# acoustic-warfare/zybo-rt-sampler-image-detection

Measured on AMD Instinct MI355X. Metric: beam-steered frames/sec (64 mics x 256 samples x 101x101 angles), higher is better.
Workload: dtype f32

## Files before the change

include/beamformer_hip.h:

```cpp
#ifndef BEAMFORMER_HIP_H
#define BEAMFORMER_HIP_H

#include <stdbool.h>

#ifdef __cplusplus
extern "C" {
#endif


void pad_delay(float *signal, float *out, int pos_pad);
void miso_pad(float *signals, float *out, int *adaptive_array, int n, int offset);
void miso_pad2(float *signals, float *out, int *adaptive_array, int n, int offset);
void mimo_pad(float *signals, float *image, int *adaptive_array, int n);
void load_coefficients_pad(int *whole_samples, int n);
void load_coefficients_pad2(int *whole_miso, int n);
void unload_coefficients_pad(void);
void unload_coefficients_pad2(void);

void lerp_delay(float *signal, float *out, float h, int pad);
void miso_lerp(float *signals, float *out, int *adaptive_array, int n, int offset);
void mimo_lerp(float *signals, float *image, int *adaptive_array, int n);
void load_coefficients_lerp(float *delays, int n);
void unload_coefficients_lerp(void);

// ... 32 lines not shown


enum bf_algo {
    BF_PAD = 0,
    BF_LERP = 1,
    BF_HYBRID = 2,
    BF_FIR_NAIVE = 3,
    BF_FIR_VEC = 4
};

int bf_configure(int n_microphones, int n_samples, int max_res_x, int max_res_y, int n_taps);
int bf_configure_from_json(const char *path);
void bf_get_config(int out[5]);

const char *bf_last_error(void);
void bf_clear_error(void);

int bf_gpu_available(void);
int bf_last_das_variant(void);
int bf_last_das_reloads(long long *changes, long long *steps);
int bf_sweep_order(const int *whole, int n_dirs, int n_mics, int dir_begin, int dir_end, int dpw, int *order_out);
int bf_read_phase_stamps(unsigned long long *out16, int clear);
int bf_read_wave_stamps(unsigned long long *out128, int clear);
int bf_set_device(int device);

void bf_publish_frame(const float *signals);
int bf_miso_listen_block(float *out, float mic_gain);
int bf_get_steer(int *n_out);

int bf_das_device(int algo, const float *d_signals, int m_total, float *d_images, int image_stride, int frames,
                  const int *adaptive_array, int n, int dir_begin, int dir_end, void *stream);

int bf_miso_device(int algo, const float *d_signals, int m_total, int frames, const int *adaptive_array, int n,
                   const int *d_offsets, int beams, float mic_gain, float *d_out, int out_stride, int *d_status, void *stream);
int bf_peak_offsets_device(const float *d_power, int frames, int image_stride, int n_dirs, int offset_per_dir,
                           int *d_offsets, void *stream);

#define BF_PEAKS_MAX_K 64
int bf_peaks_device(const float *d_power, int frames, int image_stride, int rows, int cols, int radius, int k,
                    float floor_rel, float floor_abs, int offset_per_dir,
                    int *d_offsets, float *d_values, int *d_counts, void *stream);

#define BF_REMOVE_MAX_BEAMS 64
int bf_remove_sources_device(int algo, const float *d_signals, int m_total, int frames, const int *adaptive_array, int n,
                             const int *d_offsets, int beams, const float *d_beams, int beam_stride, float gain,
                             float *d_residual, int *d_status, void *stream);
// ... 153 lines not shown
```

zybo-rt-sampler-image-detection_amd/csrc/beamformer_api.cpp:

```cpp
#include <hip/hip_runtime.h>

#include <algorithm>
#include <chrono>
#include <cmath>
#include <cstdarg>
#include <cstdio>
#include <cstdlib>
#include <cstring>
#include <initializer_list>
#include <limits>
#include <mutex>
#include <string>
#include <thread>
#include <vector>

#include "../../include/beamformer_hip.h"
#include "das_kernels.h"
#include "sweep_order.h"

namespace {

using bf::Algo;

struct Sizes {
// ... 748 lines not shown
{
    if (!need_ptrs("bf_sweep_order", {{whole, "whole"}, {order_out, "order_out"}})) return -1;
    if (n_dirs < 1 || n_mics < 1 || dpw < 1 || dir_begin < 0 || dir_end > n_dirs || dir_begin >= dir_end) {
        set_error("bf_sweep_order: want n_dirs, n_mics, dpw >= 1 and 0 <= dir_begin < dir_end <= n_dirs (got %d, %d, %d, [%d, %d))", n_dirs, n_mics, dpw,
                  dir_begin, dir_end);
        return -1;
    }
    static_assert(sizeof(int) == sizeof(int32_t), "the C-ABI's int tables are int32");
    return bf::sweep_order(reinterpret_cast<const int32_t*>(whole) + (size_t)dir_begin * n_mics, n_mics, dir_end - dir_begin, n_mics, dir_begin, dpw,
                           reinterpret_cast<int32_t*>(order_out), nullptr);
}
int bf_read_phase_stamps(unsigned long long* out16, int clear)
{
    std::lock_guard<std::mutex> lock(S().mu);
    if (!out16 || !ensure_device()) return -1;
    return HIP_OK(hipDeviceSynchronize()) && HIP_OK(bf::read_phase_stamps(out16, clear != 0)) ? 0 : -1;
}
int bf_read_wave_stamps(unsigned long long* out128, int clear)
{
    std::lock_guard<std::mutex> lock(S().mu);
    if (!out128 || !ensure_device()) return -1;
    return HIP_OK(hipDeviceSynchronize()) && HIP_OK(bf::read_wave_stamps(out128, clear != 0)) ? 0 : -1;
}

int bf_gpu_available(void)
{
    int count = 0;
    return (hipGetDeviceCount(&count) == hipSuccess && count > 0) ? 1 : 0;
}

int bf_set_device(int device)
{
    std::lock_guard<std::mutex> lock(S().mu);
    if (S().device_ready && device != S().device) { set_error("bf_set_device: device %d already in use", S().device); return -1; }
    S().device = device;
    return 0;
}


void load_coefficients_pad(int* whole_samples, int n) { (void)load_whole_only(SLOT_PAD, whole_samples, n, "load_coefficients_pad"); }
void unload_coefficients_pad(void) { std::lock_guard<std::mutex> lock(S().mu); S().tab[SLOT_PAD].drop(); }

void load_coefficients_pad2(int* whole_miso, int n)
{
    std::lock_guard<std::mutex> lock(S().mu);
    if (!whole_miso || n < 1) { set_error("load_coefficients_pad2: null or empty table"); return; }
// ... 1134 lines not shown
```

zybo-rt-sampler-image-detection_amd/csrc/das_device.h:

```cpp
#pragma once
#include "das_geometry.h"

namespace bf {

namespace {

struct KArgs {
    long long miso_row;
    int n_mics, m_total, n_samples, n_taps;
    int dir_begin, dir_end, image_stride, image_origin;
    int lead, row_stride, mic_chunk, n_chunks, tile_dirs, n_tiles;
    int scratch_off, srow, pbw;
    int n_is_pow2;
    float inv_n;
    int n_frames;
    int wg_frames, frame_inner;
    long long digest_h_off;
    long long digest_t_off;
    long long digest_o_off;
};

__device__ __forceinline__ void tile_and_frame(const KArgs& a, int* tile, int* frame)
{
    const unsigned id = blockIdx.x;
    if (a.frame_inner) {
        const unsigned x = id & 7u, j = id >> 3;
        *tile = (int)(x + 8u * (j / (unsigned)a.wg_frames));
        *frame = (int)(j % (unsigned)a.wg_frames);
    } else {
        *tile = (int)(id % (unsigned)a.n_tiles);
        *frame = (int)(id / (unsigned)a.n_tiles);
    }
}

#define BF_TABLE_PARAMS                                                                                   \
    const float* __restrict__ signals, float* __restrict__ images, const int32_t* __restrict__ mics,     \
        const int32_t* __restrict__ whole, const float* __restrict__ frac, const float* __restrict__ taps
#define BF_TABLE_ARGS signals, images, mics, whole, frac, taps

__device__ __forceinline__ float wave_sum(float v)
{
#pragma unroll
    for (int off = 32; off > 0; off >>= 1) v += __shfl_xor(v, off, kWave);
    return v;
}

__device__ __forceinline__ void stage_chunk(float* lds, const KArgs& a, const int32_t* __restrict__ mics,
                                            const float* __restrict__ frame, int m0, int mc, int wave, int nwaves, int lane)
{
    const int n = a.n_samples;
    for (int r = wave; r < mc; r += nwaves) {
        const int mic = mics[m0 + r];
        const float* src = frame + (size_t)mic * n;
        float* dst = lds + r * a.row_stride + a.lead;
        if ((n & 3) == 0) {
            const float4* s4 = reinterpret_cast<const float4*>(src);
// ... 193 lines not shown
```

zybo-rt-sampler-image-detection_amd/csrc/das_kernels.h:

```cpp
#pragma once
#include <hip/hip_runtime.h>
#include <stdint.h>

namespace bf {

enum Algo : int {
    ALGO_PAD = 0,
    ALGO_LERP = 1,
    ALGO_HYBRID = 2,
    ALGO_FIR_NAIVE = 3,
    ALGO_FIR_VEC = 4,
    ALGO_COUNT = 5
};

struct DeviceTables {
    const int32_t* whole = nullptr;
    const float* frac = nullptr;
    const float* taps = nullptr;
    int max_whole = 0;
    bool digest_direct = false;
    const int32_t* digest = nullptr;
    long long digest_order_off = 0;
};

// ... 120 lines not shown
hipError_t launch_mvdr_learn(const float* d_signals, int m_total, int frames, int n_samples, const int32_t* d_mics, int n, int seg_first, int seg_hop, int segs,
                             const double* d_window, const double* d_weights, double forget, const double* d_tau, int dirs, const int32_t* d_offsets, int sources,
                             int offset_per_dir, int n_taps, int bin_lo, int bin_hi, double loading, double* d_acc, double* d_mass, int32_t* d_used,
                             double* d_snap, double* d_cov, double* d_chol, double* d_gains, float* d_taps, int32_t* d_status, int32_t* d_fallback,
                             hipStream_t stream);

hipError_t launch_fd_steering(const double* d_tau, const double* d_freq, int n_dirs, int n_mics, int n_bins, float* d_are, float* d_aim, hipStream_t stream);
size_t fd_twiddle_floats(int n_samples, int n_bins);
hipError_t launch_fd_twiddles(int n_samples, int bin_lo, int n_bins, float* d_tw, hipStream_t stream);
hipError_t launch_fd_dft(const float* d_frames, const int32_t* d_mics, int m_total, int n_samples, int n_frames, int n_mics, int bin_lo, int n_bins,
                         const float* d_tw, float* xre_mf, float* xim_mf, float* xre_fm, float* xim_fm, hipStream_t stream);
size_t fd_workspace_floats(int n_rows, int n_dirs, int n_bins);
hipError_t launch_fd_das_power(const float* xre_mf, const float* xim_mf, const float* are, const float* aim, int n_frames, int n_mics, int n_dirs,
                               int n_bins, float* d_power, float* d_work, size_t work_floats, hipStream_t stream);
hipError_t launch_fd_covariance(const float* xre_fm, const float* xim_fm, int n_frames, int n_mics, int n_bins, float* rre, float* rim, hipStream_t stream);
size_t fd_cholesky_workspace_floats(int n_mics, int n_bins);
hipError_t launch_fd_cholesky_inverse(const float* rre, const float* rim, int n_mics, int n_bins, float loading, float* lire_t, float* liim_t,
                                      int* d_status, float* d_work, size_t work_floats, hipStream_t stream);
hipError_t launch_fd_mvdr_power(const float* lire_t, const float* liim_t, const float* are, const float* aim, int n_mics, int n_dirs, int n_bins,
                                float* d_power, float* d_work, size_t work_floats, hipStream_t stream);

hipError_t read_phase_stamps(unsigned long long* out16, bool clear);
hipError_t read_wave_stamps(unsigned long long* out128, bool clear);

hipError_t launch_yolo_decode(const void* const raw[3], const int hs[3], const int ws[3], const int strides[3], const float* anchors,
                              int batch, int nc, int format, float conf_thres, float* d_boxes, float* d_scores, int* d_cls, hipStream_t stream);
hipError_t launch_upsample_concat(const void* a, const void* b, void* out, int B, int H, int W, int ca, int cb, int elem_bytes, hipStream_t stream);
hipError_t launch_sppf_pool(void* buf, int B, int H, int W, int c, int elem_bytes, hipStream_t stream);
hipError_t launch_preprocess_bgr8(const void* frames, void* out, long long pixels, int cpad, int elem_bytes, hipStream_t stream);
int conv_dma_switch(int value);
int conv_f32_mode(int value);
int gemm_f32_mode(int value);
int conv_weight_row(int elem_bytes, int kh, int kw, int c);
hipError_t launch_conv2d_nhwc(int elem_bytes, const void* x, const void* w, const float* bias, void* y, int B, int H, int W, int C, int N, int KH, int KW,
                              int stride, int pad, int act, int ldy, const void* res, int ldr, const void* x2, int c1, int ld1, int ld2, int up1,
                              hipStream_t stream);
hipError_t launch_topk_candidates(const float* d_scores, const float* d_boxes, const int* d_cls, int batch, int total, int K, float* d_top_scores,
                                  float* d_top_boxes, int* d_top_cls, int* d_counts, hipStream_t stream);
hipError_t launch_nms(const float* d_boxes, const float* d_scores, const int* d_cls, const int* d_counts, int batch, int K, float iou_thres,
                      int max_det, unsigned long long* d_mask, float* d_out, int* d_out_count, hipStream_t stream);

}
```

zybo-rt-sampler-image-detection_amd/csrc/das_pair.hip:

```cpp
#include "das_device.h"

namespace bf {

namespace {

namespace copies {


#define BF_P_ACC(n, j, f) [a##n##0] "+v"(acc[j][f][0]), [a##n##1] "+v"(acc[j][f][1])
#define BF_P_PAD_STEP(n0, n1)                                                                             \
    "v_pk_add_f32 %[a" #n0 "0], %[a" #n0 "0], %[s0l]\n\tv_pk_add_f32 %[a" #n0 "1], %[a" #n0 "1], %[s0h]\n\t" \
    "v_pk_add_f32 %[a" #n1 "0], %[a" #n1 "0], %[s1l]\n\tv_pk_add_f32 %[a" #n1 "1], %[a" #n1 "1], %[s1h]\n\t"
#define BF_P_PAD_READ                                                                                     \
    "ds_read_b64 %[s0l], %[ad] offset:0\n\tds_read_b64 %[s0h], %[ad] offset:8\n\t"                         \
    "ds_read_b64 %[s1l], %[ad] offset:%[f0]\n\tds_read_b64 %[s1h], %[ad] offset:%[f8]\n\t"                 \
    "s_waitcnt lgkmcnt(0)\n\t"
#define BF_P_ADDR(e) "v_add_u32 %[ad], %[" #e "], %[lb]\n\t"
#define BF_P_CHECK(n, ep, ec) "s_cmp_lg_u32 %[" #ec "], %[" #ep "]\n\ts_cbranch_scc1 .Lr" #n "_%=\n.Lb" #n "_%=:\n\t"
#define BF_P_STUB(n, ec, READ) ".Lr" #n "_%=:\n\t" BF_P_ADDR(ec) READ "s_branch .Lb" #n "_%=\n"

__device__ __forceinline__ void pair_pad_first(f32x2 (&acc)[8][2][2], Quad& S0, Quad& S1, int eb, int ec, int lbase)
{
    using G = PairGeo;
    int ad;
// ... 11 lines not shown

__device__ __forceinline__ void pair_pad_rest(f32x2 (&acc)[8][2][2], Quad& S0, Quad& S1, const int (&e)[8], int lbase)
{
    using G = PairGeo;
    int ad;
#define BF_P_ACC2(n, j) [a##n##0] "+v"(acc[j][0][0]), [a##n##1] "+v"(acc[j][0][1]), [b##n##0] "+v"(acc[j][1][0]), [b##n##1] "+v"(acc[j][1][1])
#define BF_P_PAD1(n) "v_pk_add_f32 %[a" #n "0], %[a" #n "0], %[s0l]\n\tv_pk_add_f32 %[a" #n "1], %[a" #n "1], %[s0h]\n\t" \
                     "v_pk_add_f32 %[b" #n "0], %[b" #n "0], %[s1l]\n\tv_pk_add_f32 %[b" #n "1], %[b" #n "1], %[s1h]\n\t"
    asm volatile(BF_P_CHECK(2, e1, e2) BF_P_PAD1(2) BF_P_CHECK(3, e2, e3) BF_P_PAD1(3) BF_P_CHECK(4, e3, e4) BF_P_PAD1(4)
                 BF_P_CHECK(5, e4, e5) BF_P_PAD1(5) BF_P_CHECK(6, e5, e6) BF_P_PAD1(6) BF_P_CHECK(7, e6, e7) BF_P_PAD1(7)
                 ".subsection 1\n" BF_P_STUB(2, e2, BF_P_PAD_READ) BF_P_STUB(3, e3, BF_P_PAD_READ) BF_P_STUB(4, e4, BF_P_PAD_READ)
                 BF_P_STUB(5, e5, BF_P_PAD_READ) BF_P_STUB(6, e6, BF_P_PAD_READ) BF_P_STUB(7, e7, BF_P_PAD_READ) "\t.subsection 0"
                 : BF_P_ACC2(2, 2), BF_P_ACC2(3, 3), BF_P_ACC2(4, 4), BF_P_ACC2(5, 5), BF_P_ACC2(6, 6), BF_P_ACC2(7, 7),
                   [s0l] "+v"(S0.lo), [s0h] "+v"(S0.hi), [s1l] "+v"(S1.lo), [s1h] "+v"(S1.hi), [ad] "=&v"(ad)
                 : [e1] "s"(e[1]), [e2] "s"(e[2]), [e3] "s"(e[3]), [e4] "s"(e[4]), [e5] "s"(e[5]), [e6] "s"(e[6]), [e7] "s"(e[7]), [lb] "v"(lbase),
                   [f0] "n"(G::kFoff), [f8] "n"(G::kFoff + 8)
                 : "scc");
#undef BF_P_ACC2
#undef BF_P_PAD1
}

#ifdef BF_STAMPS
__device__ unsigned long long g_stamps[64 * 16];
#define BF_STAMP_DECL unsigned long long st_acc[8] = {0, 0, 0, 0, 0, 0, 0, 0}; unsigned long long st_prev = __builtin_amdgcn_s_memtime();
#define BF_STAMP(k) do { const unsigned long long st_now = __builtin_amdgcn_s_memtime(); st_acc[k] += st_now - st_prev; st_prev = st_now; } while (0)
__device__ unsigned long long g_wave_stamps[64 * 16 * 8];
__device__ unsigned char g_wave_simd[4096 * 16];
#define BF_STAMP_FLUSH do { if (lane == 0) { unsigned long long* gs = g_stamps + 16 * (blockIdx.x & 63); for (int i = 0; i < 8; ++i) atomicAdd(&gs[i], st_acc[i]); atomicAdd(&gs[8], 1ull); \
                            unsigned simd; asm volatile("s_getreg_b32 %0, hwreg(HW_REG_HW_ID, 4, 2)" : "=s"(simd)); \
                            unsigned long long* gw = g_wave_stamps + 128 * (blockIdx.x & 63) + 8 * (wave & 15); \
                            atomicAdd(&gw[0], st_acc[0]); atomicAdd(&gw[1], st_acc[3]); atomicAdd(&gw[2 + (simd & 3)], 1ull); \
                            g_wave_simd[16 * (blockIdx.x & 4095) + (wave & 15)] = (unsigned char)(0x80 | (simd & 3)); } } while (0)
#else
#define BF_STAMP_DECL
#define BF_STAMP(k)
#define BF_STAMP_FLUSH
#endif

template <int ALGO>
__global__ void __launch_bounds__(1024, 4) das_pair_kernel(BF_TABLE_PARAMS, KArgs a)
{
    static_assert(ALGO == ALGO_PAD, "das_pair_kernel: pad (lerp runs das_pair2_kernel)");
    using G = PairGeo;
    constexpr int C = G::kC, RS = G::kRs, LEAD = G::kLead, HC = G::kHalf, W = 16, DW = 8, kGroup = DW * W, kPark = Geo<1>::kPark;
    extern __shared__ __attribute__((aligned(16))) float lds[];
    const int lane = threadIdx.x & (kWave - 1);
    const int wave = __builtin_amdgcn_readfirstlane((int)(threadIdx.x >> 6));
    int tile, fpair;
    tile_and_frame(a, &tile, &fpair);
    const int f0 = 2 * fpair;
    const bool two = f0 + 1 < a.n_frames;
    const int f1 = two ? f0 + 1 : f0;
    const int tile_begin = a.dir_begin + tile * a.tile_dirs;
    if (tile_begin >= a.dir_end) return;
    const int tile_end = min(tile_begin + a.tile_dirs, a.dir_end);
    const int M = a.n_mics, N = a.n_samples;
    const int n_half = M / HC;
    const float* __restrict__ sig0 = signals + (size_t)f0 * a.m_total * N;
    const float* __restrict__ sig1 = signals + (size_t)f1 * a.m_total * N;
    float* __restrict__ img0 = images + (size_t)f0 * a.image_stride;
    float* __restrict__ img1 = images + (size_t)f1 * a.image_stride;
    const int32_t* __restrict__ dig = reinterpret_cast<const int32_t*>(taps);

    const int vmic = (lane < n_half) ? mics[lane * HC + (wave >> 1)] : 0;
    auto fetch = [&](int h) -> float4 {
        const int mic = (h < kWave) ? __builtin_amdgcn_readlane(vmic, h) : mics[h * HC + (wave >> 1)];
        const float* src = ((wave & 1) ? sig1 : sig0) + (size_t)mic * N;
        float4 v = make_float4(0.f, 0.f, 0.f, 0.f);
        if (4 * lane < N) v = *reinterpret_cast<const float4*>(src + 4 * lane);
        return v;
    };
    auto stage = [&](int h, const float4 v, bool wipe) {
        float* row0 = lds + (((h & 1) * W) + wave) * G::kSlot;
        const float py = dpp_prev(v.y), pz = dpp_prev(v.z), pw = dpp_prev(v.w);
        write_copies<C>(row0, RS, LEAD, lane, v, py, pz, pw);
        if (wipe) {
            static_assert((LEAD >> 2) * C <= kWave, "one lane per prefix quad");
            constexpr int PQ = LEAD >> 2;
            if (lane < PQ * C) reinterpret_cast<float4*>(row0 + (lane / PQ) * RS)[lane % PQ] = make_float4(0.f, 0.f, 0.f, 0.f);
        }
    };

    float4 st = fetch(0);
    const int lb = 16 * lane + (int)(unsigned)(size_t)((__attribute__((address_space(3))) char*)lds);
    BF_STAMP_DECL

    for (int g0 = tile_begin; g0 < tile_end; g0 += kGroup) {
        f32x2 acc[DW][2][2];
#pragma unroll
        for (int j = 0; j < DW; ++j)
#pragma unroll
            for (int f = 0; f < 2; ++f) { acc[j][f][0] = f32x2{0.0f, 0.0f}; acc[j][f][1] = f32x2{0.0f, 0.0f}; }

        BF_STAMP(7);
        __syncthreads();
        BF_STAMP(1);
        stage(0, st, true);
        st = fetch(1);
        BF_STAMP(2);
        __syncthreads();
        BF_STAMP(3);

        for (int h = 0; h < n_half; ++h) {
            asm volatile("s_setprio 3");
            if (h + 1 < n_half) {
                stage(h + 1, st, h == 0);
                if (h + 2 < n_half) st = fetch(h + 2);
                else if (g0 + kGroup < tile_end) st = fetch(0);
                BF_STAMP(2);
            }
            const int dw0 = g0 + wave * DW;
            if (dw0 < tile_end) {
                const size_t grp = (size_t)(dw0 - a.dir_begin) / DW;
                const int32_t* __restrict__ et = dig + (grp * M + (size_t)h * HC) * DW;
                struct Entries { int e[DW]; };
                auto request = [&](Entries& t, int m) {
#pragma unroll
                    for (int j = 0; j < DW; ++j) t.e[j] = et[m * DW + j];
                };
// ... 36 lines not shown
            auto park = [&](auto mul_c) {
#pragma unroll
                for (int j = 0; j < DW; ++j) {
                    float* row = lds + (wave * DW + j) * kPark;
                    const f32x2 a0 = acc[j][f][0], a1 = acc[j][f][1];
                    float o0, o1, o2, o3;
                    mic_mean<decltype(mul_c)::value>(a0.x, a0.y, a1.x, a1.y, M, a.inv_n, o0, o1, o2, o3);
                    reinterpret_cast<float4*>(row)[lane] = make_float4(o0 * o0, o1 * o1, o2 * o2, o3 * o3);
                }
            };
            if (__builtin_expect(a.n_is_pow2, 1)) park(std::true_type{}); else park(std::false_type{});
            BF_STAMP(5);
            __syncthreads();
            BF_STAMP(6);
            const int g = wave * kWave + lane;
            const int d = g0 + g;
            if (g < kGroup && d < tile_end && (f == 0 || two)) {
                const int dd = a.digest_o_off != 0 ? dig[a.digest_o_off + (d - a.dir_begin)] : d;
                (f == 0 ? img0 : img1)[dd - a.image_origin] = row_mean_power<false>(lds + g * kPark, N);
            }
        }
    }
    BF_STAMP(7);
    BF_STAMP_FLUSH;
}
#undef BF_P_ACC
#undef BF_P_PAD_STEP
#undef BF_P_PAD_READ
#undef BF_P_ADDR
#undef BF_P_CHECK
#undef BF_P_STUB


#define BF_I_ACC(n, j) [a##n##0] "+v"(acc[j][0]), [a##n##1] "+v"(acc[j][1]), [a##n##2] "+v"(acc[j][2]), [a##n##3] "+v"(acc[j][3])
#define BF_I_READ                                                                                   \
    "ds_read_b128 v[96:99], v120\n\tds_read_b128 v[100:103], v120 offset:1024\n\t"                   \
    "ds_read_b128 v[104:107], v120 offset:%[g0]\n\tds_read_b128 v[108:111], v120 offset:%[g1]\n\ts_waitcnt lgkmcnt(0)\n\t"
#define BF_I_STEP(n, h, mods)                                                                       \
    "v_pk_fma_f32 v[112:113], %[" #h "], v[104:105], v[96:97] " mods "\n\tv_pk_fma_f32 v[114:115], %[" #h "], v[106:107], v[98:99] " mods "\n\t" \
    "v_pk_fma_f32 v[116:117], %[" #h "], v[108:109], v[100:101] " mods "\n\tv_pk_fma_f32 v[118:119], %[" #h "], v[110:111], v[102:103] " mods "\n\t" \
    "v_pk_add_f32 %[a" #n "0], %[a" #n "0], v[112:113]\n\tv_pk_add_f32 %[a" #n "1], %[a" #n "1], v[114:115]\n\t" \
    "v_pk_add_f32 %[a" #n "2], %[a" #n "2], v[116:117]\n\tv_pk_add_f32 %[a" #n "3], %[a" #n "3], v[118:119]\n\t"
#define BF_I_FIRST(h, mods)                                                                         \
    "ds_read_b128 v[96:99], v120\n\tds_read_b128 v[104:107], v120 offset:%[g0]\n\t"                \
    "ds_read_b128 v[100:103], v120 offset:1024\n\tds_read_b128 v[108:111], v120 offset:%[g1]\n\ts_waitcnt lgkmcnt(2)\n\t" \
    "v_pk_fma_f32 v[112:113], %[" #h "], v[104:105], v[96:97] " mods "\n\tv_pk_fma_f32 v[114:115], %[" #h "], v[106:107], v[98:99] " mods "\n\t" \
    "v_pk_add_f32 %[a00], %[a00], v[112:113]\n\tv_pk_add_f32 %[a01], %[a01], v[114:115]\n\ts_waitcnt lgkmcnt(0)\n\t" \
// ... 25 lines not shown
                 : BF_I_ACC(1, 1), BF_I_ACC(2, 2), BF_I_ACC(3, 3), BF_I_ACC(4, 4), BF_I_ACC(5, 5), BF_I_ACC(6, 6), BF_I_ACC(7, 7)
                 : [e0] "s"(e[0]), [e1] "s"(e[1]), [e2] "s"(e[2]), [e3] "s"(e[3]), [e4] "s"(e[4]), [e5] "s"(e[5]), [e6] "s"(e[6]), [e7] "s"(e[7]), [lb] "v"(lbase),
                   [h01] "s"(hp[0]), [h23] "s"(hp[1]), [h45] "s"(hp[2]), [h67] "s"(hp[3]), [g0] "n"(G::kDoff), [g1] "n"(G::kDoff + 1024)
                 : "scc", BF_I_CLOB);
}
#undef BF_I_ACC
#undef BF_I_READ
#undef BF_I_FIRST
#undef BF_I_STEP
#undef BF_I_EVEN
#undef BF_I_ODD
#undef BF_I_CHECK
#undef BF_I_STUB
#undef BF_I_CLOB

template <int ALGO>
__global__ void __launch_bounds__(1024, 4) das_pair2_kernel(BF_TABLE_PARAMS, KArgs a)
{
    static_assert(ALGO == ALGO_LERP, "das_pair2_kernel: lerp (pad runs das_pair_kernel)");
    using G = Pair2Geo;
    constexpr int C = G::kC, RS = G::kRs, LEAD = G::kLead, HC = G::kHalf, W = 16, DW = 8, kGroup = DW * W, kParkHalf = Geo<1>::kParkHalf;
    static_assert(2 * kGroup * kParkHalf <= G::kMc * G::kSlot, "both frames' parked half rows fit the LDS image they alias");
    extern __shared__ __attribute__((aligned(16))) float lds[];
    const int lane = threadIdx.x & (kWave - 1);
    auto lane_id = []() -> int {
        int l;
        asm volatile("v_mbcnt_lo_u32_b32 %0, -1, 0\n\tv_mbcnt_hi_u32_b32 %0, -1, %0" : "=v"(l));
        return l;
    };
    const int wave = __builtin_amdgcn_readfirstlane((int)(threadIdx.x >> 6));
    int tile, fpair;
    tile_and_frame(a, &tile, &fpair);
    const int f0 = 2 * fpair;
    const bool two = f0 + 1 < a.n_frames;
    const int f1 = two ? f0 + 1 : f0;
    const int tile_begin = a.dir_begin + tile * a.tile_dirs;
    if (tile_begin >= a.dir_end) return;
    const int tile_end = min(tile_begin + a.tile_dirs, a.dir_end);
    const int M = a.n_mics, N = a.n_samples;
    const int n_half = M / HC;
    const float* __restrict__ sig0 = signals + (size_t)f0 * a.m_total * N;
    const float* __restrict__ sig1 = signals + (size_t)f1 * a.m_total * N;
    float* __restrict__ img0 = images + (size_t)f0 * a.image_stride;
    float* __restrict__ img1 = images + (size_t)f1 * a.image_stride;
    const int32_t* __restrict__ dig = reinterpret_cast<const int32_t*>(taps);

    const int my_mic = wave & 7, part = wave >> 3;
    constexpr unsigned kHalfBytes = HC * G::kSlot * 4;
    const bool full = N == 256;
    const unsigned row_bytes = 4u * (unsigned)N, hoff_end = (unsigned)n_half * (HC * 4u);
    unsigned voff = min(16u * (unsigned)lane, row_bytes - 16u);
    const bool in_row = 16u * (unsigned)lane < row_bytes;
    const char* mic_ids = reinterpret_cast<const char*>(mics + my_mic);
    unsigned hoff = 0;
    int mic_a = *reinterpret_cast<const int32_t*>(mic_ids);
    struct Staged2 { float4 v0, v1; };
    auto fetch_next = [&]() -> Staged2 {
        const size_t row = (size_t)(unsigned)mic_a * row_bytes;
        const char* r0 = reinterpret_cast<const char*>(sig0) + row;
        const char* r1 = reinterpret_cast<const char*>(sig1) + row;
        asm volatile("" : "+v"(voff));
        Staged2 st;
        st.v0 = *reinterpret_cast<const float4*>(r0 + voff);
        st.v1 = *reinterpret_cast<const float4*>(r1 + voff);
        hoff = hoff + HC * 4u < hoff_end ? hoff + HC * 4u : 0u;
        mic_a = *reinterpret_cast<const int32_t*>(mic_ids + hoff);
        return st;
    };
#define BF_I_DPP " row_mask:0xf bank_mask:0xf bound_ctrl:1\n\t"
    const int lb = 16 * lane + (int)(unsigned)(size_t)((__attribute__((address_space(3))) char*)lds);
    const int row0 = (my_mic * G::kSlot + part * C * RS) * 4 - (int)(unsigned)(size_t)((__attribute__((address_space(3))) char*)lds), row1 = row0 + (int)kHalfBytes;
    auto stage = [&](int row, const Staged2& st) {
        const int ad = 2 * lb + row;
        float4 x = st.v0, y = st.v1;
        if (!full) {
            asm volatile(";BF_STAGE_MASKED");
            x = make_float4(in_row ? x.x : 0.f, in_row ? x.y : 0.f, in_row ? x.z : 0.f, in_row ? x.w : 0.f);
            y = make_float4(in_row ? y.x : 0.f, in_row ? y.y : 0.f, in_row ? y.z : 0.f, in_row ? y.w : 0.f);
        }
        asm volatile("s_cmp_eq_u32 %[part], 0\n\ts_cbranch_scc1 .Lp0_%=\n\t"
                     "v_sub_f32 v98, %[xy], %[xx]\n\tv_sub_f32 v99, %[yy], %[yx]\n\t"
                     "v_sub_f32_dpp v104, %[xx], %[xw] wave_shl:1" BF_I_DPP "v_sub_f32_dpp v105, %[yx], %[yw] wave_shl:1" BF_I_DPP
                     "v_sub_f32 v100, %[xz], %[xy]\n\tv_sub_f32 v101, %[yz], %[yy]\n\t"
                     "v_sub_f32 v102, %[xw], %[xz]\n\tv_sub_f32 v103, %[yw], %[yz]\n"
                     ".Lst_%=:\n\t"
                     "v_mov_b32_dpp v96, v104 wave_shr:1" BF_I_DPP "v_mov_b32_dpp v97, v105 wave_shr:1" BF_I_DPP
                     "ds_write_b128 %[ad], v[98:101] offset:%[c0]\n\tds_write_b128 %[ad], v[102:105] offset:%[c0] + 16\n\t"
                     "ds_write_b128 %[ad], v[96:99] offset:%[c1]\n\tds_write_b128 %[ad], v[100:103] offset:%[c1] + 16\n\t"
                     ".subsection 1\n"
                     ".Lp0_%=:\n\t;BF_STAGE_PART0\n\t"
                     "v_mov_b32 v104, %[xw]\n\tv_mov_b32 v105, %[yw]\n\tv_mov_b32 v98, %[xx]\n\tv_mov_b32 v99, %[yx]\n\t"
                     "v_mov_b32 v100, %[xy]\n\tv_mov_b32 v101, %[yy]\n\tv_mov_b32 v102, %[xz]\n\tv_mov_b32 v103, %[yz]\n\t"
                     "s_branch .Lst_%=\n\t.subsection 0"
                     : : [xx] "v"(x.x), [xy] "v"(x.y), [xz] "v"(x.z), [xw] "v"(x.w), [yx] "v"(y.x), [yy] "v"(y.y), [yz] "v"(y.z), [yw] "v"(y.w),
                         [ad] "v"(ad), [part] "s"(part), [c0] "n"(2 * LEAD * 4), [c1] "n"((RS + 2 * LEAD) * 4)
                     : "memory", "scc", "v96", "v97", "v98", "v99", "v100", "v101", "v102", "v103", "v104", "v105");
    };
#undef BF_I_DPP
    auto wipe_prefix = [&]() {
        constexpr int PQ = LEAD >> 1;
        static_assert(2 * PQ <= kWave, "one lane per prefix quad of two rows");
        const int l = lane_id();
        if (l < 2 * PQ) {
            float* rows = lds + my_mic * G::kSlot + part * C * RS;
            float4* q = reinterpret_cast<float4*>(rows + (l < PQ ? 0 : RS)) + (l < PQ ? l : l - PQ);
            q[0] = make_float4(0.f, 0.f, 0.f, 0.f);
            *reinterpret_cast<float4*>(reinterpret_cast<char*>(q) + kHalfBytes) = make_float4(0.f, 0.f, 0.f, 0.f);
        }
    };

    BF_STAMP_DECL
    Staged2 st = fetch_next();

    for (int g0 = tile_begin; g0 < tile_end; g0 += kGroup) {
        f32x2 acc[DW][4];
#pragma unroll
        for (int j = 0; j < DW; ++j)
#pragma unroll
            for (int q = 0; q < 4; ++q) acc[j][q] = f32x2{0.0f, 0.0f};

        BF_STAMP(7);
        __syncthreads();
        BF_STAMP(1);
        wipe_prefix();
        stage(row0, st);
        st = fetch_next();
        BF_STAMP(2);
        __syncthreads();
        BF_STAMP(3);

        const int dw0 = g0 + wave * DW;
        const bool busy = dw0 < tile_end;
        const size_t grp = busy ? (size_t)(dw0 - a.dir_begin) / DW : 0;
        const int32_t* __restrict__ etg = dig + grp * M * DW;
        const float* __restrict__ htg = reinterpret_cast<const float*>(dig) + a.digest_h_off + grp * M * DW;
        int row_next = row1;
        for (int h = 0; h < n_half; ++h) {
            asm volatile("s_setprio 3");
            asm volatile(";BF_STAGE_BEGIN");
            if (h + 1 < n_half) {
                stage(row_next, st);
                row_next = row0 + row1 - row_next;
                st = fetch_next();
                BF_STAMP(2);
            }
            asm volatile(";BF_STAGE_END");
// ... 14 lines not shown
                    constexpr int K = decltype(kc)::value, K2 = (K + 2) % 3;
                    const Entries& cur = E[K];
                    pair2_first(acc, cur.e[0], cur.hp[0], lb);
                    request(E[K2], m + 2);
                    pair2_rest(acc, cur.e, cur.hp, lb);
                };
                using I0 = std::integral_constant<int, 0>; using I1 = std::integral_constant<int, 1>; using I2 = std::integral_constant<int, 2>;
                static_assert(HC == 8, "eight mics, the three entry sets in rotation");
                mic(0, I0{}); mic(1, I1{});
                asm volatile("s_setprio 2");
                mic(2, I2{}); mic(3, I0{});
                asm volatile("s_setprio 1");
                mic(4, I1{}); mic(5, I2{});
                asm volatile("s_setprio 0");
                mic(6, I0{}); mic(7, I1{});
                __builtin_amdgcn_s_waitcnt(0xC07F);
            }
            BF_STAMP(0);
            __syncthreads();
            BF_STAMP(h + 1 < n_half ? 3 : 4);
        }
        asm volatile("s_setprio 0");

        auto power_pass = [&](auto mul_c) __attribute__((always_inline)) {
        constexpr bool MUL = decltype(mul_c)::value;
        if constexpr (MUL) asm volatile(";BF_POWER_POW2"); else asm volatile(";BF_POWER_DIV");
        int wv = wave;
        asm volatile("" : "+s"(wv));
        float sum = 0.0f;
#pragma unroll
        for (int r = 0; r < 2; ++r) {
            if (r == 1) {
                __syncthreads();
                BF_STAMP(4);
            }
            {
                auto squares = [&](int j, f32x2& s0, f32x2& s1) __attribute__((always_inline)) {
                    if constexpr (MUL) {
                        const f32x2 inv2 = {a.inv_n, a.inv_n};
                        s0 = acc[j][2 * r] * inv2; s1 = acc[j][2 * r + 1] * inv2;
                    } else {
                        float o0, o1, o2, o3;
                        mic_mean<false>(acc[j][2 * r].x, acc[j][2 * r + 1].x, acc[j][2 * r].y, acc[j][2 * r + 1].y, M, a.inv_n, o0, o1, o2, o3);
                        s0 = f32x2{o0, o2}; s1 = f32x2{o1, o3};
                    }
                    s0 = s0 * s0; s1 = s1 * s1;
// ... 15 lines not shown
                    park2(ad, s0, s1, t0, t1, std::false_type{});
                    park2(ad + kGroup * kParkHalf * 4u, s0, s1, t0, t1, std::true_type{});
                }
            }
            BF_STAMP(5);
            __syncthreads();
            BF_STAMP(6);
            if (wv < 2 * (kGroup / kWave)) {
                const int lane_o = lane_id();
                const int g = (wv & 1) * kWave + lane_o;
                const int d = g0 + g;
                if (d < tile_end && (wv < kGroup / kWave || two)) {
                    const unsigned row = (unsigned)(size_t)((__attribute__((address_space(3))) char*)lds) + (unsigned)(wv * kWave + lane_o) * (kParkHalf * 4u);
                    sum = add_in_order_rolling(row, r == 0 ? 32 : (N - 128) >> 2, sum);
                    if (r == 1) {
                        const int dd = a.digest_o_off != 0 ? dig[a.digest_o_off + (d - a.dir_begin)] : d;
                        (wv < kGroup / kWave ? img0 : img1)[dd - a.image_origin] = sum / (float)N;
                    }
                }
            }
        }
        asm volatile(";BF_POWER_END");
        };
        if (__builtin_expect(a.n_is_pow2, 1)) power_pass(std::true_type{}); else power_pass(std::false_type{});
    }
    BF_STAMP(7);
    BF_STAMP_FLUSH;
}

}

template <int ALGO>
hipError_t launch_pair_algo(const DasLaunch& L, const DasPlan& plan, int frames, hipStream_t stream)
{
    constexpr bool kLerp = ALGO == ALGO_LERP;
    using PG = std::conditional_t<kLerp, copies::Pair2Geo, copies::PairGeo>;
    if (L.tab.digest_direct || plan.waves != copies::kWaves || plan.mic_chunk != PG::kMc || plan.row_stride != PG::kRs ||
        plan.lead != PG::kLead || plan.interleaved != (kLerp ? 1 : 0) || (L.n_mics % 16) != 0)
        return hipErrorInvalidValue;
    auto kernel = [] { if constexpr (kLerp) return copies::das_pair2_kernel<ALGO>; else return copies::das_pair_kernel<ALGO>; }();
    static int pair_scratch = -1;
    const dim3 pair_grid((unsigned)plan.n_tiles * (unsigned)((frames + 1) / 2));
    return launch_with_lds(kernel, pair_grid, dim3((unsigned)plan.waves * kWave), plan.lds_bytes, stream, &pair_scratch, L.signals, L.images, L.mics,
                           L.tab.whole, L.tab.frac, reinterpret_cast<const float*>(L.tab.digest), make_args(L, plan));
}

}

hipError_t launch_pair(const DasLaunch& L, const DasPlan& plan, int frames, hipStream_t stream)
{
    switch (L.algo) {
        case ALGO_PAD: return launch_pair_algo<ALGO_PAD>(L, plan, frames, stream);
        case ALGO_LERP: return launch_pair_algo<ALGO_LERP>(L, plan, frames, stream);
        default: return hipErrorInvalidValue;
    }
}

hipError_t read_phase_stamps(unsigned long long* out16, bool clear)
{
#ifdef BF_STAMPS
    static unsigned long long all[64 * 16];
    hipError_t e = hipMemcpyFromSymbol(all, HIP_SYMBOL(copies::g_stamps), sizeof(all));
    if (e != hipSuccess) return e;
    for (int i = 0; i < 16; ++i) { out16[i] = 0; for (int r = 0; r < 64; ++r) out16[i] += all[16 * r + i]; }
    if (!clear) return e;
    for (int i = 0; i < 64 * 16; ++i) all[i] = 0;
    return hipMemcpyToSymbol(HIP_SYMBOL(copies::g_stamps), all, sizeof(all));
#else
    for (int i = 0; i < 16; ++i) out16[i] = 0;
// ... 12 lines not shown
    static unsigned char simd[4096 * 16];
    e = hipMemcpyFromSymbol(simd, HIP_SYMBOL(copies::g_wave_simd), sizeof(simd));
    if (e != hipSuccess) return e;
    for (int g = 0; g < 4096; ++g) {
        const unsigned char* s = simd + 16 * g;
        bool whole = true;
        for (int w = 0; w < 16; ++w) whole = whole && (s[w] & 0x80);
        if (!whole) continue;
        for (int w = 0; w < 16; ++w) { out128[8 * w + 6] += s[w] == s[w & 3]; out128[8 * w + 7] += 1; }
    }
    if (!clear) return e;
    for (int i = 0; i < 64 * 128; ++i) all[i] = 0;
    for (int i = 0; i < 4096 * 16; ++i) simd[i] = 0;
    e = hipMemcpyToSymbol(HIP_SYMBOL(copies::g_wave_simd), simd, sizeof(simd));
    if (e != hipSuccess) return e;
    return hipMemcpyToSymbol(HIP_SYMBOL(copies::g_wave_stamps), all, sizeof(all));
#else
    for (int i = 0; i < 128; ++i) out128[i] = 0;
    (void)clear;
    return hipSuccess;
#endif
}

}
```

zybo-rt-sampler-image-detection_amd/lib/_native.py:

```python
import ctypes as C
import os

import numpy as np

_HERE = os.path.dirname(os.path.abspath(__file__))
LIB_PATH = os.environ.get("BF_NATIVE_LIB") or os.path.join(_HERE, "libbeamformer_hip.so")


class BeamformerError(RuntimeError):
    """An entry point of libbeamformer_hip.so reported a failure (bf_last_error)."""


if not os.path.exists(LIB_PATH):
    raise ImportError("%s is missing: build it with `python -c 'import __graft_entry__ as g; g.build()'` "
                      "(hipcc --offload-arch=gfx950).  There is no CPU fallback." % LIB_PATH)

if os.environ.get("BF_NO_TORCH", "0") != "1":
    try:
        import torch
    except Exception:
        pass

lib = C.CDLL(LIB_PATH)

# ... 40 lines not shown
_sig("convolve_hybrid_delay_add", None, FP, FP, C.c_int, FP)
_sig("get_data", None, FP)
for _n in ("pad_mimo", "lerp_mimo", "convolve_mimo_naive", "convolve_mimo_vectorized", "mimo_truncated"):
    _sig(_n, None, FP, IP, C.c_int)
_sig("miso_steer_listen", None, FP, IP, C.c_int, C.c_int)
_sig("load", C.c_int, C.c_bool)
for _n in ("stop_receiving", "signal_handler", "stop_miso"):
    _sig(_n, None)
_sig("load_miso", C.c_int)
_sig("load_pa", None, IP, C.c_int)
_sig("steer", None, C.c_int)
_sig("bf_configure", C.c_int, C.c_int, C.c_int, C.c_int, C.c_int, C.c_int)
_sig("bf_configure_from_json", C.c_int, C.c_char_p)
_sig("bf_get_config", None, IP)
_sig("bf_last_error", C.c_char_p)
_sig("bf_clear_error", None)
_sig("bf_gpu_available", C.c_int)
_sig("bf_last_das_variant", C.c_int)
_sig("bf_last_das_reloads", C.c_int, C.POINTER(C.c_longlong), C.POINTER(C.c_longlong))
_sig("bf_sweep_order", C.c_int, IP, C.c_int, C.c_int, C.c_int, C.c_int, C.c_int, IP)
_sig("bf_set_device", C.c_int, C.c_int)
_sig("bf_read_phase_stamps", C.c_int, C.POINTER(C.c_ulonglong), C.c_int)
_sig("bf_read_wave_stamps", C.c_int, C.POINTER(C.c_ulonglong), C.c_int)
_sig("bf_publish_frame", None, FP)
_sig("bf_miso_listen_block", C.c_int, FP, C.c_float)
_sig("bf_get_steer", C.c_int, IP)
_sig("bf_das_device", C.c_int, C.c_int, C.c_void_p, C.c_int, C.c_void_p, C.c_int, C.c_int, IP, C.c_int, C.c_int, C.c_int, C.c_void_p)
_sig("bf_miso_device", C.c_int, C.c_int, C.c_void_p, C.c_int, C.c_int, IP, C.c_int, C.c_void_p, C.c_int, C.c_float, C.c_void_p, C.c_int, C.c_void_p,
     C.c_void_p)
_sig("bf_remove_sources_device", C.c_int, C.c_int, C.c_void_p, C.c_int, C.c_int, IP, C.c_int, C.c_void_p, C.c_int, C.c_void_p, C.c_int, C.c_float, C.c_void_p,
     C.c_void_p, C.c_void_p)
_sig("bf_stream_history", C.c_int, C.c_int)
_sig("bf_miso_stream_device", C.c_int, C.c_int, C.c_void_p, C.c_int, C.c_int, C.c_int, C.c_void_p, IP, C.c_int, C.c_void_p, C.c_int, C.c_float, C.c_void_p,
     C.c_int, C.c_void_p, C.c_void_p)
_sig("bf_das_stream_device", C.c_int, C.c_int, C.c_void_p, C.c_int, C.c_void_p, C.c_int, C.c_int, C.c_int, C.c_void_p, IP, C.c_int, C.c_int, C.c_int,
     C.c_void_p)
_sig("bf_peak_offsets_device", C.c_int, C.c_void_p, C.c_int, C.c_int, C.c_int, C.c_int, C.c_void_p, C.c_void_p)
_sig("bf_peaks_device", C.c_int, C.c_void_p, C.c_int, C.c_int, C.c_int, C.c_int, C.c_int, C.c_int, C.c_float, C.c_float, C.c_int, C.c_void_p, C.c_void_p,
     C.c_void_p, C.c_void_p)
_sig("bf_track_state_words", C.c_int, C.c_int)
_sig("bf_track_sources_device", C.c_int, C.c_void_p, C.c_int, C.c_int, C.c_int, C.c_int, C.c_int, C.c_int, C.c_float, C.c_int, C.c_int, C.c_float, C.c_float,
     C.c_void_p, C.c_void_p, C.c_void_p, C.c_void_p, C.c_void_p, C.c_void_p, C.c_void_p)
_sig("bf_fuse_boxes_device", C.c_int, C.c_void_p, C.c_int, C.c_int, C.c_int, C.c_int, C.c_int, C.c_void_p, C.c_void_p, C.c_int, C.c_int, C.c_int, C.c_float,
     C.c_void_p, C.c_int, C.c_void_p, C.c_void_p, C.c_void_p, C.c_void_p, C.c_void_p, C.c_void_p, C.c_void_p)
_sig("bf_box_track_state_words", C.c_int, C.c_int)
_sig("bf_track_boxes_device", C.c_int, C.c_void_p, C.c_void_p, C.c_int, C.c_int, C.c_float, C.c_int, C.c_float, C.c_int, C.c_int, C.c_void_p, C.c_void_p,
# ... 138 lines not shown
```

Before: 146,700.

## Make pair DAS kernels persistent with a CU-sized grid-stride work loop

The pair beamforming kernels now launch a grid capped at the CU count (rounded down to a multiple of 8), and each workgroup loops over tile/frame-pair items with a grid stride read from the implicit kernel arguments. Per-item signal and image pointers are rebuilt from the kernarg segment on every iteration. The goal is to cut workgroup launch and tail overhead and to keep LDS setup resident across items. The trade-off is lower occupancy, since only one workgroup runs per CU with 1024-thread blocks, and possible load imbalance across CUs. A per-item timestamp probe and a runtime grid-cap knob are also added.

```diff
diff --git a/include/beamformer_hip.h b/include/beamformer_hip.h
--- a/include/beamformer_hip.h
+++ b/include/beamformer_hip.h
@@ -78,6 +78,8 @@
 int bf_sweep_order(const int *whole, int n_dirs, int n_mics, int dir_begin, int dir_end, int dpw, int *order_out);
 int bf_read_phase_stamps(unsigned long long *out16, int clear);
 int bf_read_wave_stamps(unsigned long long *out128, int clear);
+int bf_read_item_stamps(unsigned long long *out, int n_items, int clear);
+int bf_pair_grid_cap(int cap);
 int bf_set_device(int device);
 
 void bf_publish_frame(const float *signals);
diff --git a/zybo-rt-sampler-image-detection_amd/csrc/beamformer_api.cpp b/zybo-rt-sampler-image-detection_amd/csrc/beamformer_api.cpp
--- a/zybo-rt-sampler-image-detection_amd/csrc/beamformer_api.cpp
+++ b/zybo-rt-sampler-image-detection_amd/csrc/beamformer_api.cpp
@@ -794,6 +794,13 @@
     if (!out128 || !ensure_device()) return -1;
     return HIP_OK(hipDeviceSynchronize()) && HIP_OK(bf::read_wave_stamps(out128, clear != 0)) ? 0 : -1;
 }
+int bf_read_item_stamps(unsigned long long* out, int n_items, int clear)
+{
+    std::lock_guard<std::mutex> lock(S().mu);
+    if (!out || n_items < 1 || n_items > 4096 || !ensure_device()) return -1;
+    return HIP_OK(hipDeviceSynchronize()) && HIP_OK(bf::read_item_stamps(out, n_items, clear != 0)) ? 0 : -1;
+}
+int bf_pair_grid_cap(int cap) { return bf::pair_grid_cap(cap < 0 ? 0 : cap); }
 
 int bf_gpu_available(void)
 {
diff --git a/zybo-rt-sampler-image-detection_amd/csrc/das_device.h b/zybo-rt-sampler-image-detection_amd/csrc/das_device.h
--- a/zybo-rt-sampler-image-detection_amd/csrc/das_device.h
+++ b/zybo-rt-sampler-image-detection_amd/csrc/das_device.h
@@ -20,9 +20,8 @@
     long long digest_o_off;
 };
 
-__device__ __forceinline__ void tile_and_frame(const KArgs& a, int* tile, int* frame)
-{
-    const unsigned id = blockIdx.x;
+__device__ __forceinline__ void tile_and_frame(const KArgs& a, unsigned id, int* tile, int* frame)
+{
     if (a.frame_inner) {
         const unsigned x = id & 7u, j = id >> 3;
         *tile = (int)(x + 8u * (j / (unsigned)a.wg_frames));
@@ -32,6 +31,7 @@
         *frame = (int)(id / (unsigned)a.n_tiles);
     }
 }
+__device__ __forceinline__ void tile_and_frame(const KArgs& a, int* tile, int* frame) { tile_and_frame(a, blockIdx.x, tile, frame); }
 
 #define BF_TABLE_PARAMS                                                                                   \
     const float* __restrict__ signals, float* __restrict__ images, const int32_t* __restrict__ mics,     \
diff --git a/zybo-rt-sampler-image-detection_amd/csrc/das_kernels.h b/zybo-rt-sampler-image-detection_amd/csrc/das_kernels.h
--- a/zybo-rt-sampler-image-detection_amd/csrc/das_kernels.h
+++ b/zybo-rt-sampler-image-detection_amd/csrc/das_kernels.h
@@ -166,6 +166,8 @@
 
 hipError_t read_phase_stamps(unsigned long long* out16, bool clear);
 hipError_t read_wave_stamps(unsigned long long* out128, bool clear);
+hipError_t read_item_stamps(unsigned long long* out, int n_items, bool clear);
+int pair_grid_cap(int cap);
 
 hipError_t launch_yolo_decode(const void* const raw[3], const int hs[3], const int ws[3], const int strides[3], const float* anchors,
                               int batch, int nc, int format, float conf_thres, float* d_boxes, float* d_scores, int* d_cls, hipStream_t stream);
diff --git a/zybo-rt-sampler-image-detection_amd/csrc/das_pair.hip b/zybo-rt-sampler-image-detection_amd/csrc/das_pair.hip
--- a/zybo-rt-sampler-image-detection_amd/csrc/das_pair.hip
+++ b/zybo-rt-sampler-image-detection_amd/csrc/das_pair.hip
@@ -57,21 +57,71 @@
 
 #ifdef BF_STAMPS
 __device__ unsigned long long g_stamps[64 * 16];
-#define BF_STAMP_DECL unsigned long long st_acc[8] = {0, 0, 0, 0, 0, 0, 0, 0}; unsigned long long st_prev = __builtin_amdgcn_s_memtime();
+#define BF_STAMP_DECL unsigned long long st_acc[8] = {0, 0, 0, 0, 0, 0, 0, 0}; unsigned long long st_prev = __builtin_amdgcn_s_memtime(); \
+                      unsigned long long mk_first = st_prev, mk_sync = 0;
 #define BF_STAMP(k) do { const unsigned long long st_now = __builtin_amdgcn_s_memtime(); st_acc[k] += st_now - st_prev; st_prev = st_now; } while (0)
+#define BF_STAMP_SYNC do { if (mk_sync == 0) mk_sync = st_prev; } while (0)
 __device__ unsigned long long g_wave_stamps[64 * 16 * 8];
 __device__ unsigned char g_wave_simd[4096 * 16];
-#define BF_STAMP_FLUSH do { if (lane == 0) { unsigned long long* gs = g_stamps + 16 * (blockIdx.x & 63); for (int i = 0; i < 8; ++i) atomicAdd(&gs[i], st_acc[i]); atomicAdd(&gs[8], 1ull); \
-                            unsigned simd; asm volatile("s_getreg_b32 %0, hwreg(HW_REG_HW_ID, 4, 2)" : "=s"(simd)); \
-                            unsigned long long* gw = g_wave_stamps + 128 * (blockIdx.x & 63) + 8 * (wave & 15); \
+__device__ unsigned long long g_item_marks[4096 * 4];
+#define BF_STAMP_FLUSH(id) do { if (lane == 0) { unsigned long long* gs = g_stamps + 16 * ((id) & 63); for (int i = 0; i < 8; ++i) atomicAdd(&gs[i], st_acc[i]); atomicAdd(&gs[8], 1ull); \
+                            unsigned hw, xcc; asm volatile("s_getreg_b32 %0, hwreg(HW_REG_HW_ID)\n\ts_getreg_b32 %1, hwreg(HW_REG_XCC_ID, 0, 4)" : "=s"(hw), "=s"(xcc)); \
+                            const unsigned simd = hw >> 4; \
+                            unsigned long long* gw = g_wave_stamps + 128 * ((id) & 63) + 8 * (wave & 15); \
                             atomicAdd(&gw[0], st_acc[0]); atomicAdd(&gw[1], st_acc[3]); atomicAdd(&gw[2 + (simd & 3)], 1ull); \
-                            g_wave_simd[16 * (blockIdx.x & 4095) + (wave & 15)] = (unsigned char)(0x80 | (simd & 3)); } } while (0)
+                            g_wave_simd[16 * ((id) & 4095) + (wave & 15)] = (unsigned char)(0x80 | (simd & 3)); \
+                            if (wave == 0) { unsigned long long* gm = g_item_marks + 4 * ((id) & 4095); gm[0] = mk_first; gm[1] = mk_sync; gm[2] = st_prev; \
+                                             gm[3] = 1ull << 63 | (unsigned long long)(xcc << 16 | (hw & 0xff00u)); } } \
+                            for (int i = 0; i < 8; ++i) st_acc[i] = 0; \
+                            st_prev = __builtin_amdgcn_s_memtime(); mk_first = st_prev; mk_sync = 0; } while (0)
 #else
 #define BF_STAMP_DECL
 #define BF_STAMP(k)
-#define BF_STAMP_FLUSH
+#define BF_STAMP_SYNC
+#define BF_STAMP_FLUSH(id)
 #endif
 
+struct PairParams { const float* signals; float* images; const int32_t* mics; const int32_t* whole; const float* frac; const float* taps; KArgs a; };
+__device__ __forceinline__ const __attribute__((address_space(4))) PairParams* pair_params()
+{
+    auto* p = (const __attribute__((address_space(4))) PairParams*)__builtin_amdgcn_kernarg_segment_ptr();
+    asm volatile("" : "+s"(p));
+    return p;
+}
+__device__ __forceinline__ KArgs pair_item_args(const __attribute__((address_space(4))) PairParams* p)
+{
+    KArgs a{};
+    a.n_tiles = p->a.n_tiles; a.wg_frames = p->a.wg_frames; a.frame_inner = p->a.frame_inner; a.n_frames = p->a.n_frames;
+    a.dir_begin = p->a.dir_begin; a.dir_end = p->a.dir_end; a.tile_dirs = p->a.tile_dirs;
+    a.image_stride = p->a.image_stride; a.m_total = p->a.m_total; a.n_samples = p->a.n_samples;
+    return a;
+}
+__device__ __forceinline__ unsigned pair_stride()
+{
+    using CP = const __attribute__((address_space(4))) char*;
+    const auto off = (CP)__builtin_amdgcn_implicitarg_ptr() - (CP)__builtin_amdgcn_kernarg_segment_ptr();
+    return *(const __attribute__((address_space(4))) unsigned*)((CP)pair_params() + off);
+}
+struct PairItem { int tile_begin, tile_end, two; const float* sig0; const float* sig1; float* img0; float* img1; };
+__device__ __forceinline__ int pair_item(unsigned id, PairItem& it)
+{
+    const auto* p = pair_params();
+    const KArgs a = pair_item_args(p);
+    if (id >= (unsigned)a.n_tiles * (unsigned)a.wg_frames) return -1;
+    int tile, fpair;
+    tile_and_frame(a, id, &tile, &fpair);
+    it.tile_begin = a.dir_begin + tile * a.tile_dirs;
+    if (it.tile_begin >= a.dir_end) return 0;
+    it.tile_end = min(it.tile_begin + a.tile_dirs, a.dir_end);
+    const int f0 = 2 * fpair;
+    it.two = f0 + 1 < a.n_frames;
+    const int f1 = it.two ? f0 + 1 : f0;
+    it.sig0 = p->signals + (size_t)f0 * a.m_total * a.n_samples;
+    it.sig1 = p->signals + (size_t)f1 * a.m_total * a.n_samples;
+    it.img0 = p->images + (size_t)f0 * a.image_stride;
+    it.img1 = p->images + (size_t)f1 * a.image_stride;
+    return 1;
+}
 template <int ALGO>
 __global__ void __launch_bounds__(1024, 4) das_pair_kernel(BF_TABLE_PARAMS, KArgs a)
 {
@@ -79,23 +129,14 @@
     using G = PairGeo;
     constexpr int C = G::kC, RS = G::kRs, LEAD = G::kLead, HC = G::kHalf, W = 16, DW = 8, kGroup = DW * W, kPark = Geo<1>::kPark;
     extern __shared__ __attribute__((aligned(16))) float lds[];
+    BF_STAMP_DECL
     const int lane = threadIdx.x & (kWave - 1);
     const int wave = __builtin_amdgcn_readfirstlane((int)(threadIdx.x >> 6));
-    int tile, fpair;
-    tile_and_frame(a, &tile, &fpair);
-    const int f0 = 2 * fpair;
-    const bool two = f0 + 1 < a.n_frames;
-    const int f1 = two ? f0 + 1 : f0;
-    const int tile_begin = a.dir_begin + tile * a.tile_dirs;
-    if (tile_begin >= a.dir_end) return;
-    const int tile_end = min(tile_begin + a.tile_dirs, a.dir_end);
     const int M = a.n_mics, N = a.n_samples;
     const int n_half = M / HC;
-    const float* __restrict__ sig0 = signals + (size_t)f0 * a.m_total * N;
-    const float* __restrict__ sig1 = signals + (size_t)f1 * a.m_total * N;
-    float* __restrict__ img0 = images + (size_t)f0 * a.image_stride;
-    float* __restrict__ img1 = images + (size_t)f1 * a.image_stride;
     const int32_t* __restrict__ dig = reinterpret_cast<const int32_t*>(taps);
+    const float* sig0 = signals;
+    const float* sig1 = signals;
 
     const int vmic = (lane < n_half) ? mics[lane * HC + (wave >> 1)] : 0;
     auto fetch = [&](int h) -> float4 {
@@ -116,9 +157,19 @@
         }
     };
 
-    float4 st = fetch(0);
     const int lb = 16 * lane + (int)(unsigned)(size_t)((__attribute__((address_space(3))) char*)lds);
-    BF_STAMP_DECL
+    float4 st = make_float4(0.f, 0.f, 0.f, 0.f);
+    for (unsigned id = blockIdx.x;; id += pair_stride()) {
+    PairItem it;
+    const int have = pair_item(id, it);
+    if (have < 0) break;
+    if (have == 0) continue;
+    sig0 = it.sig0; sig1 = it.sig1;
+    st = fetch(0);
+    const int tile_begin = it.tile_begin, tile_end = it.tile_end;
+    const bool two = it.two != 0;
+    float* __restrict__ img0 = it.img0;
+    float* __restrict__ img1 = it.img1;
 
     for (int g0 = tile_begin; g0 < tile_end; g0 += kGroup) {
         f32x2 acc[DW][2][2];
@@ -130,6 +181,7 @@
         BF_STAMP(7);
         __syncthreads();
         BF_STAMP(1);
+        BF_STAMP_SYNC;
         stage(0, st, true);
         st = fetch(1);
         BF_STAMP(2);
@@ -212,7 +264,8 @@
         }
     }
     BF_STAMP(7);
-    BF_STAMP_FLUSH;
+    BF_STAMP_FLUSH(id);
+    }
 }
 #undef BF_P_ACC
 #undef BF_P_PAD_STEP
@@ -284,6 +337,7 @@
     constexpr int C = G::kC, RS = G::kRs, LEAD = G::kLead, HC = G::kHalf, W = 16, DW = 8, kGroup = DW * W, kParkHalf = Geo<1>::kParkHalf;
     static_assert(2 * kGroup * kParkHalf <= G::kMc * G::kSlot, "both frames' parked half rows fit the LDS image they alias");
     extern __shared__ __attribute__((aligned(16))) float lds[];
+    BF_STAMP_DECL
     const int lane = threadIdx.x & (kWave - 1);
     auto lane_id = []() -> int {
         int l;
@@ -291,21 +345,11 @@
         return l;
     };
     const int wave = __builtin_amdgcn_readfirstlane((int)(threadIdx.x >> 6));
-    int tile, fpair;
-    tile_and_frame(a, &tile, &fpair);
-    const int f0 = 2 * fpair;
-    const bool two = f0 + 1 < a.n_frames;
-    const int f1 = two ? f0 + 1 : f0;
-    const int tile_begin = a.dir_begin + tile * a.tile_dirs;
-    if (tile_begin >= a.dir_end) return;
-    const int tile_end = min(tile_begin + a.tile_dirs, a.dir_end);
     const int M = a.n_mics, N = a.n_samples;
     const int n_half = M / HC;
-    const float* __restrict__ sig0 = signals + (size_t)f0 * a.m_total * N;
-    const float* __restrict__ sig1 = signals + (size_t)f1 * a.m_total * N;
-    float* __restrict__ img0 = images + (size_t)f0 * a.image_stride;
-    float* __restrict__ img1 = images + (size_t)f1 * a.image_stride;
     const int32_t* __restrict__ dig = reinterpret_cast<const int32_t*>(taps);
+    const float* sig0 = signals;
+    const float* sig1 = signals;
 
     const int my_mic = wave & 7, part = wave >> 3;
     constexpr unsigned kHalfBytes = HC * G::kSlot * 4;
@@ -314,21 +358,26 @@
     unsigned voff = min(16u * (unsigned)lane, row_bytes - 16u);
     const bool in_row = 16u * (unsigned)lane < row_bytes;
     const char* mic_ids = reinterpret_cast<const char*>(mics + my_mic);
-    unsigned hoff = 0;
-    int mic_a = *reinterpret_cast<const int32_t*>(mic_ids);
+    unsigned hoff = HC * 4u;
+    int mic_a = *reinterpret_cast<const int32_t*>(mic_ids + hoff);
     struct Staged2 { float4 v0, v1; };
-    auto fetch_next = [&]() -> Staged2 {
-        const size_t row = (size_t)(unsigned)mic_a * row_bytes;
+    auto fetch_rows = [&](int mic) -> Staged2 {
+        const size_t row = (size_t)(unsigned)mic * row_bytes;
         const char* r0 = reinterpret_cast<const char*>(sig0) + row;
         const char* r1 = reinterpret_cast<const char*>(sig1) + row;
         asm volatile("" : "+v"(voff));
         Staged2 st;
         st.v0 = *reinterpret_cast<const float4*>(r0 + voff);
         st.v1 = *reinterpret_cast<const float4*>(r1 + voff);
+        return st;
+    };
+    auto fetch_next = [&]() -> Staged2 {
+        const Staged2 st = fetch_rows(mic_a);
         hoff = hoff + HC * 4u < hoff_end ? hoff + HC * 4u : 0u;
         mic_a = *reinterpret_cast<const int32_t*>(mic_ids + hoff);
         return st;
     };
+    auto fetch_first = [&]() -> Staged2 { return fetch_rows(*reinterpret_cast<const int32_t*>(mic_ids)); };
 #define BF_I_DPP " row_mask:0xf bank_mask:0xf bound_ctrl:1\n\t"
     const int lb = 16 * lane + (int)(unsigned)(size_t)((__attribute__((address_space(3))) char*)lds);
     const int row0 = (my_mic * G::kSlot + part * C * RS) * 4 - (int)(unsigned)(size_t)((__attribute__((address_space(3))) char*)lds), row1 = row0 + (int)kHalfBytes;
@@ -371,8 +420,19 @@
         }
     };
 
-    BF_STAMP_DECL
-    Staged2 st = fetch_next();
+    Staged2 st{};
+    for (unsigned id = blockIdx.x;; id += pair_stride()) {
+    PairItem it;
+    const int have = pair_item(id, it);
+    if (have < 0) break;
+    if (have == 0) continue;
+    sig0 = it.sig0; sig1 = it.sig1;
+    st = fetch_first();
+    const int tile_begin = it.tile_begin, tile_end = it.tile_end;
+    int two_i = __builtin_amdgcn_readfirstlane(it.two);
+    asm volatile("" : "+s"(two_i));
+    float* __restrict__ img0 = it.img0;
+    float* __restrict__ img1 = it.img1;
 
     for (int g0 = tile_begin; g0 < tile_end; g0 += kGroup) {
         f32x2 acc[DW][4];
@@ -384,6 +444,7 @@
         BF_STAMP(7);
         __syncthreads();
         BF_STAMP(1);
+        BF_STAMP_SYNC;
         wipe_prefix();
         stage(row0, st);
         st = fetch_next();
@@ -444,6 +505,9 @@
         }
         asm volatile("s_setprio 0");
 
+        int two_here = two_i;
+        asm volatile("" : "+s"(two_here));
+        const bool two = two_here != 0;
         auto power_pass = [&](auto mul_c) __attribute__((always_inline)) {
         constexpr bool MUL = decltype(mul_c)::value;
         if constexpr (MUL) asm volatile(";BF_POWER_POW2"); else asm volatile(";BF_POWER_DIV");
@@ -505,10 +569,13 @@
         }
         asm volatile(";BF_POWER_END");
         };
-        if (__builtin_expect(a.n_is_pow2, 1)) power_pass(std::true_type{}); else power_pass(std::false_type{});
+        int pow2 = a.n_is_pow2;
+        asm volatile("" : "+s"(pow2));
+        if (__builtin_expect(pow2, 1)) power_pass(std::true_type{}); else power_pass(std::false_type{});
     }
     BF_STAMP(7);
-    BF_STAMP_FLUSH;
+    BF_STAMP_FLUSH(id);
+    }
 }
 
 }
@@ -523,11 +590,24 @@
         return hipErrorInvalidValue;
     auto kernel = [] { if constexpr (kLerp) return copies::das_pair2_kernel<ALGO>; else return copies::das_pair_kernel<ALGO>; }();
     static int pair_scratch = -1;
-    const dim3 pair_grid((unsigned)plan.n_tiles * (unsigned)((frames + 1) / 2));
+    static const unsigned n_cus = [] {
+        int dev = 0, v = 0;
+        return hipGetDevice(&dev) == hipSuccess && hipDeviceGetAttribute(&v, hipDeviceAttributeMultiprocessorCount, dev) == hipSuccess && v > 0 ? (unsigned)v : 256u;
+    }();
+    const unsigned n_items = (unsigned)plan.n_tiles * (unsigned)((frames + 1) / 2), cap = (unsigned)pair_grid_cap(-1);
+    const dim3 pair_grid(std::min(n_items, cap > 0 ? cap : std::max(n_cus & ~7u, 1u)));
     return launch_with_lds(kernel, pair_grid, dim3((unsigned)plan.waves * kWave), plan.lds_bytes, stream, &pair_scratch, L.signals, L.images, L.mics,
                            L.tab.whole, L.tab.frac, reinterpret_cast<const float*>(L.tab.digest), make_args(L, plan));
 }
 
+}
+
+int pair_grid_cap(int cap)
+{
+    static int state = 0;
+    const int old = state;
+    if (cap >= 0) state = cap;
+    return old;
 }
 
 hipError_t launch_pair(const DasLaunch& L, const DasPlan& plan, int frames, hipStream_t stream)
@@ -586,4 +666,21 @@
 #endif
 }
 
-}
+hipError_t read_item_stamps(unsigned long long* out, int n_items, bool clear)
+{
+#ifdef BF_STAMPS
+    static unsigned long long all[4096 * 4];
+    hipError_t e = hipMemcpyFromSymbol(all, HIP_SYMBOL(copies::g_item_marks), sizeof(all));
+    if (e != hipSuccess) return e;
+    for (int i = 0; i < 4 * n_items; ++i) out[i] = i < 4096 * 4 ? all[i] : 0;
+    if (!clear) return e;
+    for (int i = 0; i < 4096 * 4; ++i) all[i] = 0;
+    return hipMemcpyToSymbol(HIP_SYMBOL(copies::g_item_marks), all, sizeof(all));
+#else
+    for (int i = 0; i < 4 * n_items; ++i) out[i] = 0;
+    (void)clear;
+    return hipSuccess;
+#endif
+}
+
+}
diff --git a/zybo-rt-sampler-image-detection_amd/lib/_native.py b/zybo-rt-sampler-image-detection_amd/lib/_native.py
--- a/zybo-rt-sampler-image-detection_amd/lib/_native.py
+++ b/zybo-rt-sampler-image-detection_amd/lib/_native.py
@@ -86,6 +86,8 @@
 _sig("bf_set_device", C.c_int, C.c_int)
 _sig("bf_read_phase_stamps", C.c_int, C.POINTER(C.c_ulonglong), C.c_int)
 _sig("bf_read_wave_stamps", C.c_int, C.POINTER(C.c_ulonglong), C.c_int)
+_sig("bf_read_item_stamps", C.c_int, C.POINTER(C.c_ulonglong), C.c_int, C.c_int)
+_sig("bf_pair_grid_cap", C.c_int, C.c_int)
 _sig("bf_publish_frame", None, FP)
 _sig("bf_miso_listen_block", C.c_int, FP, C.c_float)
 _sig("bf_get_steer", C.c_int, IP)
```

After: 147,300 (median of 6 runs). Within noise of the previous version (+0.4%).
